# ETH3D/badslam

Measured on AMD Instinct MI355X. Metric: BA iterations/sec (and ms/iter) at N keyframes x M surfels, 640x480, higher is better.
Workload: dtype f32

## Files before the change

badslam_amd/csrc/kernels_surfel.hip:

```cpp
#include <stdlib.h>
#include <cstdio>

#include "ba_device.h"
#include "ba_launch.h"
#include "wave_cull.h"

namespace bahip {

#ifndef BAHIP_WAVES_ATTR
#define BAHIP_WAVES_ATTR __attribute__((amdgpu_waves_per_eu(4)))
#endif
constexpr int kSurfelBlock = 64;
constexpr int kMaxSumClasses = 8;

enum SumsMode { kSumsFused = 0, kSumsProduce = 1, kSumsConsume = 2 };
__device__ __forceinline__ bool position_valid(Vec3 p) { return p.x == p.x; }
static inline unsigned grid_for(uint32_t n) { return xcd_padded_tiles((n + kSurfelBlock - 1) / kSurfelBlock); }
#if defined(BAHIP_TILE_TIMELINE) && !defined(BAHIP_FAST_MATH)
__device__ unsigned long long g_geometry_timeline[65536][2];
void geometry_timeline_dump(const char* path) {
  static unsigned long long host[65536][2];
  if (hipMemcpyFromSymbol(host, HIP_SYMBOL(g_geometry_timeline), sizeof(host)) != hipSuccess) return;
  if (FILE* f = fopen(path, "wb")) { fwrite(host, sizeof(host), 1, f); fclose(f); }
}
#define BAHIP_RECORD_GEOMETRY_TIMELINE 1
#endif
}

BAHIP_FLAVOURED_BEGIN

template <int kWaves, int kCount, int kMode = kSumsFused, typename Visit>
__device__ __forceinline__ void tile_sums(float (&tot)[kCount], float* lds, Visit visit, int classes, const ClassPartials& cp = ClassPartials{},
                                          uint32_t i = 0, bool in_range = false) {
  static_assert(kWaves == 1 || kWaves == 2 || kWaves == 4, "1, 2 or 4 wavefronts per tile");
  static_assert(kMode == kSumsFused || kWaves == 1, "the class partials are exchanged by the one-wavefront shape only");
  if (kMode == kSumsProduce) {
#pragma nounroll
    for (int c = 0; c < classes; ++c) {
      if (!((cp.owned >> c) & 1u)) continue;
      float acc[kCount];
#pragma unroll
      for (int q = 0; q < kCount; ++q) acc[q] = 0.f;
      visit(acc, c);
      if (in_range) {
#pragma unroll
        for (int q = 0; q < kCount; ++q) cp.data[(size_t)(c * kCount + q) * cp.stride + i] = acc[q];
      }
    }
#pragma unroll
    for (int q = 0; q < kCount; ++q) tot[q] = 0.f;
  } else if (kMode == kSumsConsume) {
#pragma unroll
    for (int q = 0; q < kCount; ++q) {
      float t = cp.data[(size_t)(0 * kCount + q) * cp.stride + i] + cp.data[(size_t)(1 * kCount + q) * cp.stride + i];
      for (int c = 2; c < classes; ++c) t += cp.data[(size_t)(c * kCount + q) * cp.stride + i];
      tot[q] = t;
    }
  } else if (kWaves == 1) {
#pragma unroll
    for (int q = 0; q < kCount; ++q) tot[q] = 0.f;
#pragma nounroll
    for (int c = 0; c < classes; ++c) {
      float acc[kCount];
#pragma unroll
      for (int q = 0; q < kCount; ++q) acc[q] = 0.f;
      visit(acc, c);
#pragma unroll
      for (int q = 0; q < kCount; ++q) tot[q] += acc[q];
    }
  } else {
    const int part = threadIdx.x >> 6, lane = threadIdx.x & 63;
#pragma nounroll
    for (int c = part; c < classes; c += kWaves) {
      float acc[kCount];
#pragma unroll
      for (int q = 0; q < kCount; ++q) acc[q] = 0.f;
      visit(acc, c);
#pragma unroll
      for (int q = 0; q < kCount; ++q) lds[(c * kCount + q) * 64 + lane] = acc[q];
    }
    __syncthreads();
#pragma unroll
    for (int q = 0; q < kCount; ++q) {
      float t = lds[(0 * kCount + q) * 64 + lane] + lds[(1 * kCount + q) * 64 + lane];
      for (int c = 2; c < classes; ++c) t += lds[(c * kCount + q) * 64 + lane];
      tot[q] = t;
    }
    __syncthreads();
  }
}

__global__ void __launch_bounds__(kSurfelBlock) BAHIP_WAVES_ATTR
activation_kernel(Intrinsics in, const KfEntry* __restrict__ kfs, int num_kfs, SurfelsView s, uint32_t surfels_size) {
  const uint32_t i = xcd_chunked_tile(blockIdx.x) * kSurfelBlock + threadIdx.x;
  const bool in_range = i < surfels_size;
  const uint32_t ii = in_range ? i : 0;
  const Vec3 gp = surfel_position(s, ii);
  const Vec3 gn = surfel_normal(s, ii);
  const WaveBounds wb = wave_bounds(gp, in_range && position_valid(gp));
  bool active = false;
  for_each_candidate_until(
      num_kfs,
      [&](int k) { return kfs[k].activation == BAHIP_KF_ACTIVE && sphere_may_project(in, kfs[k].pose.F, wb); },
      [&](int k) {
        if (in_range && !active) {
          Assoc r;
          if (project_associate<false>(in, kfs[k].pose.F, kfs[k].geom, gp, gn, &r, nullptr)) active = true;
        }
        return __all(active || !in_range) != 0;
      });
  if (in_range) s.active[i] = (s.active[i] & (uint8_t)~kSurfelActiveFlag) | (active ? kSurfelActiveFlag : 0);
}

constexpr int kMaskChunks = 4;
template <int kWaves, bool kActivate, int kMode = kSumsFused>
__device__ __forceinline__ void normals_pass(const Intrinsics& in, const KfEntry* __restrict__ kfs, int num_kfs,
                                             const WaveBounds& wb, SurfelsView& s, uint32_t i, bool* live_inout, bool decide,
                                             Vec3 gp, Vec3* gn_inout, float* lds, const ClassPartials& cp = ClassPartials{},
                                             bool in_range = false, unsigned long long* masks = nullptr) {
  const bool writer = kWaves == 1 || (threadIdx.x >> 6) == 0;
  const Vec3 gn = *gn_inout;
  bool live = *live_inout;
  constexpr int kCount = kActivate ? 5 : 4;
  float sum[kCount];
  tile_sums<kWaves, kCount, kMode>(sum, lds, [&](float (&acc)[kCount], int cls) {
    struct Started { Projected p; PixelWords pix; };
    for_each_candidate_pipelined<Started>(
        num_kfs,
        [&](int k) {
          float f[12];
          int32_t activation;
          load_candidate(kfs[k].pose.F, &kfs[k].activation, f, &activation);
          return activation != BAHIP_KF_INACTIVE && sphere_may_project(in, f, wb);
        },
        [&](int k) {
          Started st;
          st.p = project_surfel(in, kfs[k].pose.F, gp);
          st.pix = load_pixel_words(in, kfs[k].geom, st.p);
          return st;
        },
        [&](int k, const Started& st) {
          const Projected& p = st.p;
          const PixelWords& pix = st.pix;
          Assoc r;
          const bool associated = live && associate_from_words<false>(in, kfs[k].pose.F, gn, p, pix, &r, nullptr);
          gathers_arrived(pix);
          if (associated) {
            const Vec3 g = mul33(kfs[k].pose.GR, unpack_normal8(r.normal_bits));
            acc[0] += g.x; acc[1] += g.y; acc[2] += g.z; acc[3] += 1.f;
            if (kActivate) acc[kCount - 1] += (kfs[k].activation == BAHIP_KF_ACTIVE) ? 1.f : 0.f;
          }
        },
        in.sum_classes, cls, masks ? masks + cls * kMaskChunks : nullptr, masks ? kMaskChunks : 0, false);
  }, in.sum_classes, cp, i, in_range);
  if (kMode == kSumsProduce) return;
  if (kActivate && decide) {
    const bool active = live && sum[kCount - 1] >= 1.f;
    if (writer) s.active[i] = (s.active[i] & (uint8_t)~kSurfelActiveFlag) | (active ? kSurfelActiveFlag : 0);
    live = active;
    *live_inout = active;
  }
  if (!live) return;
  const float sx = sum[0], sy = sum[1], sz = sum[2], count = sum[3];
  if (count >= 1) {
    const uint32_t packed = pack_normal10((1.f / count) * mk3(sx, sy, sz));
    if (writer) reinterpret_cast<uint32_t*>(s.row(kSurfelNormal))[i] = packed;
    *gn_inout = unpack_normal10(packed);
  }
}

template <int kWaves>
__global__ void __launch_bounds__(64 * kWaves) BAHIP_WAVES_ATTR
normals_kernel(Intrinsics in, const KfEntry* __restrict__ kfs, int num_kfs, SurfelsView s) {
  __shared__ float lds[kWaves == 1 ? 1 : kMaxSumClasses * 4 * 64];
  const int lane = threadIdx.x & 63;
  const uint32_t i = xcd_chunked_tile(blockIdx.x) * kSurfelBlock + lane;
  const bool in_range = i < s.size;
  const uint32_t ii = in_range ? i : 0;
  bool live = in_range && (s.active[ii] & kSurfelActiveFlag);
  const Vec3 gp = surfel_position(s, ii);
  Vec3 gn = surfel_normal(s, ii);
  const WaveBounds wb = wave_bounds(gp, live && position_valid(gp));
  normals_pass<kWaves, false>(in, kfs, num_kfs, wb, s, ii, &live, false, gp, &gn, lds);
}

template <bool kUseDepth, bool kUseDesc, int kWaves, bool kActivate, int kPhase>
__device__ __forceinline__ void geometry_step(const Intrinsics& in, const KfEntry* __restrict__ kfs, int num_kfs, SurfelsView& s,
                                              uint32_t activate_count, float* lds, const ClassPartials& cpn, const ClassPartials& cpp,
                                              uint32_t tile , unsigned long long* replay_masks) {
  constexpr int kNormalsMode = kPhase == 1 ? kSumsProduce : kPhase == 2 ? kSumsConsume : kSumsFused;
  constexpr int kPositionMode = kPhase == 2 ? kSumsProduce : kPhase == 3 ? kSumsConsume : kSumsFused;
  const int lane = threadIdx.x & 63;
  const bool writer = kWaves == 1 || (threadIdx.x >> 6) == 0;
  const uint32_t i = tile * kSurfelBlock + lane;
  const bool in_range = i < s.size;
  const uint32_t ii = in_range ? i : 0;
  const bool decide = kActivate && kPhase != 3 && in_range && i < activate_count;
  bool live = in_range && (decide || (s.active[ii] & kSurfelActiveFlag));
  const Vec3 gp = surfel_position(s, ii);
  Vec3 gn = surfel_normal(s, ii);
  const WaveBounds wb = wave_bounds(gp, live && position_valid(gp));
  if (wb.r < 0.f) {
    if (decide && writer && kPhase != 1) s.active[ii] = s.active[ii] & (uint8_t)~kSurfelActiveFlag;
    return;
  }
  constexpr bool kReplayMasks = kWaves == 1 && kPhase == 0;
  unsigned long long* masks = kReplayMasks ? replay_masks : nullptr;
  if (kPhase != 3) normals_pass<kWaves, kActivate, kNormalsMode>(in, kfs, num_kfs, wb, s, ii, &live, decide, gp, &gn, lds, cpn, in_range, masks);
  if (kPhase == 1) return;

  auto cand = [&](int k) {
    float f[12];
    int32_t activation;
    load_candidate(kfs[k].pose.F, &kfs[k].activation, f, &activation);
    return activation != BAHIP_KF_INACTIVE && sphere_may_project(in, f, wb);
  };

  if (!kUseDesc) {
    float hb[2];
    tile_sums<kWaves, 2, kPositionMode>(hb, lds, [&](float (&acc)[2], int cls) {
      for_each_candidate_cached(num_kfs, cand, [&](int k) {
        const Projected p = project_surfel(in, kfs[k].pose.F, gp);
        const PixelWords pix = load_pixel_words(in, kfs[k].geom, p);
        Assoc r;
        const bool associated = live && associate_from_words<false>(in, kfs[k].pose.F, gn, p, pix, &r, nullptr);
        gathers_arrived(pix);
        if (!associated) return;
        const float inv_std = assoc_inv_std(in, r);
        const float jac = -inv_std;
        const Vec3 u = assoc_unproject(r);
        const float raw = inv_std * dot3(r.nl, u - r.local);
        const float w = depth_residual_weight(raw);
        const float wj = w * jac;
        acc[0] = mad(wj, jac, acc[0]);
        acc[1] = mad(wj, raw, acc[1]);
      }, in.sum_classes, cls, masks ? masks + cls * kMaskChunks : nullptr, masks ? kMaskChunks : 0, masks != nullptr);
    }, in.sum_classes, cpp, ii, in_range);
    if (kPhase == 2 || !live || !writer) return;
    const float H = hb[0], b = hb[1];
    if (H > 1e-6f) {
      const float t = -1.f * b / H;
      const Vec3 np = gp + t * gn;
      s.row(kSurfelX)[i] = np.x; s.row(kSurfelY)[i] = np.y; s.row(kSurfelZ)[i] = np.z;
    }
    return;
  }

  const float radius_sq = s.row(kSurfelRadiusSquared)[ii];
  const float d1 = s.row(kSurfelDescriptor1)[ii];
  const float d2 = s.row(kSurfelDescriptor2)[ii];
  const TangentPoints tp = surfel_tangent_points(gp, gn, radius_sq);
  float tot[8];
  tile_sums<kWaves, 8, kPositionMode>(tot, lds, [&](float (&acc)[8], int cls) {
    float &a0 = acc[0], &a1 = acc[1], &a2 = acc[2], &a3 = acc[3], &a5 = acc[4], &a6 = acc[5], &a7 = acc[6], &a8 = acc[7];
    struct StartedPair { Projected p; PixelWords pix; };
    auto start_pair = [&](int k) {
      StartedPair st;
      st.p = project_surfel(in, kfs[k].pose.F, gp);
      st.pix = load_pixel_words(in, kfs[k].geom, st.p);
      return st;
    };
    auto finish_pair = [&](int k, const StartedPair& st) {
      const float* F = kfs[k].pose.F;
      const Projected& p = st.p;
      const PixelWords& pix = st.pix;
      const DescWords dw = load_descriptor_words(in, kfs[k].lumafp, F, tp, p);
      Assoc r;
      const bool associated = live && associate_from_words<false>(in, F, gn, p, pix, &r, nullptr);
#ifdef BAHIP_PIN_POSITION
      gathers_arrived(pix, dw);
#endif
      if (!associated) return;
      if (kUseDepth) {
        const float inv_std = assoc_inv_std(in, r);
        const float jac = -inv_std;
        const Vec3 u = assoc_unproject(r);
        const float raw = inv_std * dot3(r.nl, u - r.local);
        const float w = depth_residual_weight(raw);
        a0 = mad(w * jac, jac, a0);
        a6 = mad(w * raw, jac, a6);
      }
      if (dw.color_ok) {
        DescEval e;
        eval_descriptor_from_words(in, kfs[k].lumafp, dw, d1, d2, &e);
        const float jp1 = jac_descriptor_surfel(r.nl, r.local, r.inv_z, e.gx1, e.gy1, in.cfx, in.cfy);
        const float jp2 = jac_descriptor_surfel(r.nl, r.local, r.inv_z, e.gx2, e.gy2, in.cfx, in.cfy);
        const float jd = -1.f;
        const float w1 = descriptor_residual_weight(e.r1);
        const float wr1 = w1 * e.r1;
        const float w2 = descriptor_residual_weight(e.r2);
        const float wr2 = w2 * e.r2;
        a0 = mad(w2 * jp2, jp2, mad(w1 * jp1, jp1, a0));
        a1 += w1 * jp1 * jd;
        a3 += w1 * jd * jd;
        a6 = mad(wr2, jp2, mad(wr1, jp1, a6));
        a7 += wr1 * jd;
        a2 += w2 * jp2 * jd;
        a5 += w2 * jd * jd;
        a8 += wr2 * jd;
      }
    };
    if (kWaves == 1)
      for_each_candidate_pipelined<StartedPair>(num_kfs, cand, start_pair, finish_pair, in.sum_classes, cls, masks ? masks + cls * kMaskChunks : nullptr,
                                                masks ? kMaskChunks : 0, masks != nullptr);
    else
      for_each_candidate_cached(num_kfs, cand, [&](int k) { finish_pair(k, start_pair(k)); }, in.sum_classes, cls,
                                masks ? masks + cls * kMaskChunks : nullptr, masks ? kMaskChunks : 0, masks != nullptr);
  }, in.sum_classes, cpp, ii, in_range);
  if (kPhase == 2 || !live || !writer) return;
  const float a0 = tot[0], a1 = tot[1], a2 = tot[2], a3 = tot[3], a5 = tot[4], a6 = tot[5], a7 = tot[6], a8 = tot[7];

  float H00 = a0 + 1e-6f, H01 = a1, H02 = a2, H11 = a3 + 1e-6f, H12 = 0.f, H22 = a5 + 1e-6f;
  H00 = sqrtf(H00);
  H01 = H01 / H00;
  H11 = sqrtf(H11 - H01 * H01);
  H02 = H02 / H00;
  H12 = (H12 - H02 * H01) / H11;
  H22 = sqrtf(H22 - H02 * H02 - H12 * H12);
  const float y0 = a6 / H00;
  const float y1 = (a7 - H01 * y0) / H11;
  const float y2 = (a8 - H02 * y0 - H12 * y1) / H22;
  const float x2 = y2 / H22;
  const float x1 = (y1 - H12 * x2) / H11;
  const float x0 = (y0 - H02 * x2 - H01 * x1) / H00;
  if (x0 != 0) {
    const Vec3 np = gp - x0 * gn;
    s.row(kSurfelX)[i] = np.x; s.row(kSurfelY)[i] = np.y; s.row(kSurfelZ)[i] = np.z;
  }
  if (x1 != 0) s.row(kSurfelDescriptor1)[i] = fmaxf(-180.f, fminf(180.f, d1 - x1));
  if (x2 != 0) s.row(kSurfelDescriptor2)[i] = fmaxf(-180.f, fminf(180.f, d2 - x2));
}


template <bool kUseDepth, bool kUseDesc, int kWaves, bool kActivate>
__global__ void __launch_bounds__(64 * kWaves) BAHIP_WAVES_ATTR
geometry_kernel(Intrinsics in, const KfEntry* __restrict__ kfs, int num_kfs, SurfelsView s, uint32_t activate_count,
                const uint32_t* __restrict__ sched, const int* __restrict__ stop ) {
  __shared__ float lds[kWaves == 1 ? 1 : kMaxSumClasses * 8 * 64];
  __shared__ unsigned long long candidate_masks[kWaves == 1 ? kMaxSumClasses * kMaskChunks : 1];
  if (stop && load_global(stop) != 0) return;
#ifdef BAHIP_RECORD_GEOMETRY_TIMELINE
  const unsigned long long t0 = wall_clock64();
#endif
  uint32_t tile;
  if (!scheduled_tile(blockIdx.x, gridDim.x - (sched ? kHeavySlots : 0u), sched, &tile)) return;
  geometry_step<kUseDepth, kUseDesc, kWaves, kActivate, 0>(in, kfs, num_kfs, s, activate_count, lds, ClassPartials{}, ClassPartials{}, tile, candidate_masks);
#ifdef BAHIP_RECORD_GEOMETRY_TIMELINE
  if (threadIdx.x == 0 && blockIdx.x < 65536) { g_geometry_timeline[blockIdx.x][0] = t0; g_geometry_timeline[blockIdx.x][1] = wall_clock64(); }
#endif
}

#ifndef BAHIP_HYBRID_WAVES
#define BAHIP_HYBRID_WAVES 4
#endif
template <bool kUseDepth, bool kUseDesc, bool kActivate>
__global__ void __launch_bounds__(256) __attribute__((amdgpu_waves_per_eu(BAHIP_HYBRID_WAVES)))
geometry_hybrid_kernel(Intrinsics in, const KfEntry* __restrict__ kfs, int num_kfs, SurfelsView s, uint32_t activate_count,
                       const uint32_t* __restrict__ sched , uint32_t padded_tiles, const int* __restrict__ stop) {
  __shared__ float lds[kMaxSumClasses * 8 * 64];
  __shared__ unsigned long long candidate_masks[4][kMaxSumClasses * kMaskChunks];
  if (stop && load_global(stop) != 0) return;
  if (blockIdx.x < kHeavySlots) {
    if (blockIdx.x >= sched[0]) return;
    geometry_step<kUseDepth, kUseDesc, 4, kActivate, 0>(in, kfs, num_kfs, s, activate_count, lds, ClassPartials{}, ClassPartials{}, sched[8 + blockIdx.x], nullptr);
  } else {
    const uint32_t wave = threadIdx.x >> 6, position = (blockIdx.x - kHeavySlots) * 4u + wave;
    if (position >= padded_tiles) return;
    const uint32_t tile = (uint32_t)__builtin_amdgcn_readfirstlane((int)sched[kSchedPerm + position]);
    if (sched[kSchedPerm + padded_tiles + tile] != 0) return;
    geometry_step<kUseDepth, kUseDesc, 1, kActivate, 0>(in, kfs, num_kfs, s, activate_count, nullptr, ClassPartials{}, ClassPartials{}, tile, candidate_masks[wave]);
  }
}

template <bool kUseDepth, bool kUseDesc, bool kActivate, int kPhase>
__global__ void __launch_bounds__(64) BAHIP_WAVES_ATTR
geometry_phase_kernel(Intrinsics in, const KfEntry* __restrict__ kfs, int num_kfs, SurfelsView s, uint32_t activate_count,
                      ClassPartials cpn, ClassPartials cpp) {
  geometry_step<kUseDepth, kUseDesc, 1, kActivate, kPhase>(in, kfs, num_kfs, s, activate_count, nullptr, cpn, cpp, xcd_run_tile(blockIdx.x, gridDim.x), nullptr);
}

template <int kPhase>
__global__ void __launch_bounds__(kSurfelBlock) BAHIP_WAVES_ATTR
normals_phase_kernel(Intrinsics in, const KfEntry* __restrict__ kfs, int num_kfs, SurfelsView s, ClassPartials cp) {
  const uint32_t i = xcd_chunked_tile(blockIdx.x) * kSurfelBlock + threadIdx.x;
  const bool in_range = i < s.size;
  const uint32_t ii = in_range ? i : 0;
  bool live = in_range && (s.active[ii] & kSurfelActiveFlag);
  const Vec3 gp = surfel_position(s, ii);
  Vec3 gn = surfel_normal(s, ii);
  const WaveBounds wb = wave_bounds(gp, live && position_valid(gp));
  static_assert(kNormalsSums == 4, "normals_pass without activation: x, y, z, count");
  normals_pass<1, false, kPhase == 1 ? kSumsProduce : kSumsConsume>(in, kfs, num_kfs, wb, s, ii, &live, false, gp, &gn, nullptr, cp, in_range);
}

__global__ void __launch_bounds__(kSurfelBlock) BAHIP_WAVES_ATTR
activation_hits_kernel(Intrinsics in, const KfEntry* __restrict__ kfs, int num_kfs, SurfelsView s, uint32_t surfels_size,
                       uint32_t owner_mask, uint32_t owner_rank, uint32_t* __restrict__ hits) {
  const uint32_t i = xcd_chunked_tile(blockIdx.x) * kSurfelBlock + threadIdx.x;
  const bool in_range = i < surfels_size;
  const uint32_t ii = in_range ? i : 0;
  const Vec3 gp = surfel_position(s, ii);
  const Vec3 gn = surfel_normal(s, ii);
  const WaveBounds wb = wave_bounds(gp, in_range && position_valid(gp));
  bool active = false;
  for_each_candidate_until(
      num_kfs,
      [&](int k) {
        return ((uint32_t)k & owner_mask) == owner_rank && kfs[k].activation == BAHIP_KF_ACTIVE && sphere_may_project(in, kfs[k].pose.F, wb);
      },
      [&](int k) {
        if (in_range && !active) {
          Assoc r;
          if (project_associate<false>(in, kfs[k].pose.F, kfs[k].geom, gp, gn, &r, nullptr)) active = true;
        }
        return __all(active || !in_range) != 0;
      });
  if (in_range) hits[i] = active ? 1u : 0u;
}
void launch_activation(hipStream_t stream, const Intrinsics& in, const KfEntry* kfs, int num_kfs, const SurfelsView& s,
                       uint32_t surfels_size) {
  if (surfels_size == 0) return;
  hipLaunchKernelGGL(activation_kernel, dim3(grid_for(surfels_size)), dim3(kSurfelBlock), 0, stream, in, kfs, num_kfs, s,
                     surfels_size);
}

static int g_forced_tile_waves = bahip_env_int("BAHIP_TILE_WAVES", 0);
static long long g_geometry_hybrid_launches = 0;
long long geometry_hybrid_launches() { return g_geometry_hybrid_launches; }
void set_tile_waves(int waves) { g_forced_tile_waves = waves; }
static int tile_waves(uint32_t surfels) {
  const int forced = g_forced_tile_waves;
  if (forced == 1 || forced == 4) return forced;
  return grid_for(surfels) >= 8192 ? 1 : 4;
}

void launch_normals(hipStream_t stream, const Intrinsics& in, const KfEntry* kfs, int num_kfs, const SurfelsView& s) {
  if (s.size == 0) return;
  const dim3 grid(grid_for(s.size));
  switch (tile_waves(s.size)) {
    case 1: hipLaunchKernelGGL(normals_kernel<1>, grid, dim3(64), 0, stream, in, kfs, num_kfs, s); break;
    default: hipLaunchKernelGGL(normals_kernel<4>, grid, dim3(256), 0, stream, in, kfs, num_kfs, s); break;
  }
}

template <int kWaves, bool kActivate>
static void launch_geometry_shape(hipStream_t stream, bool use_depth, bool use_desc, const Intrinsics& in, const KfEntry* kfs,
                                  int num_kfs, const SurfelsView& s, uint32_t activate_count, const uint32_t* sched, const int* stop) {
  const dim3 grid(sched_positions(grid_for(s.size), sched)), block(64 * kWaves);
  if (!use_desc) hipLaunchKernelGGL((geometry_kernel<true, false, kWaves, kActivate>), grid, block, 0, stream, in, kfs, num_kfs, s, activate_count, sched, stop);
  else if (use_depth) hipLaunchKernelGGL((geometry_kernel<true, true, kWaves, kActivate>), grid, block, 0, stream, in, kfs, num_kfs, s, activate_count, sched, stop);
  else hipLaunchKernelGGL((geometry_kernel<false, true, kWaves, kActivate>), grid, block, 0, stream, in, kfs, num_kfs, s, activate_count, sched, stop);
}

template <bool kActivate>
static void launch_geometry_hybrid(hipStream_t stream, bool use_depth, bool use_desc, const Intrinsics& in, const KfEntry* kfs,
                                   int num_kfs, const SurfelsView& s, uint32_t activate_count, const uint32_t* sched, const int* stop) {
  const uint32_t padded = grid_for(s.size);
  const dim3 grid(kHeavySlots + (padded + 3u) / 4u), block(256);
  if (!use_desc) hipLaunchKernelGGL((geometry_hybrid_kernel<true, false, kActivate>), grid, block, 0, stream, in, kfs, num_kfs, s, activate_count, sched, padded, stop);
  else if (use_depth) hipLaunchKernelGGL((geometry_hybrid_kernel<true, true, kActivate>), grid, block, 0, stream, in, kfs, num_kfs, s, activate_count, sched, padded, stop);
  else hipLaunchKernelGGL((geometry_hybrid_kernel<false, true, kActivate>), grid, block, 0, stream, in, kfs, num_kfs, s, activate_count, sched, padded, stop);
}

void launch_geometry(hipStream_t stream, bool use_depth, bool use_desc, const Intrinsics& in, const KfEntry* kfs,
                     int num_kfs, const SurfelsView& s, long long activate_count, const uint32_t* sched, const int* stop) {
  if (s.size == 0) return;
  const uint32_t n = activate_count < 0 ? 0u : (uint32_t)activate_count;
  const bool hybrid = sched != nullptr && (g_forced_tile_waves == 5 || (g_forced_tile_waves == 0 && grid_for(s.size) < 8192));
  if (hybrid) {
    ++g_geometry_hybrid_launches;
    if (activate_count < 0) launch_geometry_hybrid<false>(stream, use_depth, use_desc, in, kfs, num_kfs, s, n, sched, stop);
    else launch_geometry_hybrid<true>(stream, use_depth, use_desc, in, kfs, num_kfs, s, n, sched, stop);
  } else if (tile_waves(s.size) == 1) {
    if (activate_count < 0) launch_geometry_shape<1, false>(stream, use_depth, use_desc, in, kfs, num_kfs, s, n, sched, stop);
    else launch_geometry_shape<1, true>(stream, use_depth, use_desc, in, kfs, num_kfs, s, n, sched, stop);
  } else {
    if (activate_count < 0) launch_geometry_shape<4, false>(stream, use_depth, use_desc, in, kfs, num_kfs, s, n, sched, stop);
    else launch_geometry_shape<4, true>(stream, use_depth, use_desc, in, kfs, num_kfs, s, n, sched, stop);
  }
}

template <bool kUseDepth, bool kUseDesc, bool kActivate>
static void launch_geometry_phase_of(hipStream_t stream, int phase, const Intrinsics& in, const KfEntry* kfs, int num_kfs, const SurfelsView& s,
                                     uint32_t activate_count, const ClassPartials& cpn, const ClassPartials& cpp) {
  const dim3 grid(grid_for(s.size)), block(64);
  if (phase == 1) hipLaunchKernelGGL((geometry_phase_kernel<kUseDepth, kUseDesc, kActivate, 1>), grid, block, 0, stream, in, kfs, num_kfs, s, activate_count, cpn, cpp);
  else if (phase == 2) hipLaunchKernelGGL((geometry_phase_kernel<kUseDepth, kUseDesc, kActivate, 2>), grid, block, 0, stream, in, kfs, num_kfs, s, activate_count, cpn, cpp);
  else hipLaunchKernelGGL((geometry_phase_kernel<kUseDepth, kUseDesc, kActivate, 3>), grid, block, 0, stream, in, kfs, num_kfs, s, activate_count, cpn, cpp);
}

void launch_geometry_phase(hipStream_t stream, int phase, bool use_depth, bool use_desc, const Intrinsics& in, const KfEntry* kfs, int num_kfs,
                           const SurfelsView& s, long long activate_count, const ClassPartials& cpn, const ClassPartials& cpp) {
  if (s.size == 0) return;
  const uint32_t n = activate_count < 0 ? 0u : (uint32_t)activate_count;
  const bool act = activate_count >= 0;
  if (!use_desc) {
    if (act) launch_geometry_phase_of<true, false, true>(stream, phase, in, kfs, num_kfs, s, n, cpn, cpp);
    else launch_geometry_phase_of<true, false, false>(stream, phase, in, kfs, num_kfs, s, n, cpn, cpp);
  } else if (use_depth) {
    if (act) launch_geometry_phase_of<true, true, true>(stream, phase, in, kfs, num_kfs, s, n, cpn, cpp);
    else launch_geometry_phase_of<true, true, false>(stream, phase, in, kfs, num_kfs, s, n, cpn, cpp);
  } else {
    if (act) launch_geometry_phase_of<false, true, true>(stream, phase, in, kfs, num_kfs, s, n, cpn, cpp);
    else launch_geometry_phase_of<false, true, false>(stream, phase, in, kfs, num_kfs, s, n, cpn, cpp);
  }
}

void launch_normals_phase(hipStream_t stream, int phase, const Intrinsics& in, const KfEntry* kfs, int num_kfs, const SurfelsView& s, const ClassPartials& cp) {
  if (s.size == 0) return;
  const dim3 grid(grid_for(s.size)), block(kSurfelBlock);
  if (phase == 1) hipLaunchKernelGGL(normals_phase_kernel<1>, grid, block, 0, stream, in, kfs, num_kfs, s, cp);
  else hipLaunchKernelGGL(normals_phase_kernel<2>, grid, block, 0, stream, in, kfs, num_kfs, s, cp);
}

void launch_activation_hits(hipStream_t stream, const Intrinsics& in, const KfEntry* kfs, int num_kfs, const SurfelsView& s, uint32_t surfels_size,
                            int kf_rank, int kf_world, uint32_t* hits) {
  if (surfels_size == 0) return;
  hipLaunchKernelGGL(activation_hits_kernel, dim3(grid_for(surfels_size)), dim3(kSurfelBlock), 0, stream, in, kfs, num_kfs, s, surfels_size,
                     (uint32_t)(kf_world - 1), (uint32_t)kf_rank, hits);
}
BAHIP_FLAVOURED_END

#ifndef BAHIP_FAST_MATH
namespace bahip {
__device__ __forceinline__ void sample_rgba(const uint8_t* color, uint32_t pitch, int w, int h, float x, float y, float (&out)[4]) {
  float xb = x - 0.5f, yb = y - 0.5f;
  if (!(xb >= -1.f)) xb = -1.f;
  if (xb > (float)w) xb = (float)w;
  if (!(yb >= -1.f)) yb = -1.f;
  if (yb > (float)h) yb = (float)h;
  const float fx = floorf(xb), fy = floorf(yb);
  const float a = xb - fx, b = yb - fy;
  const int x0 = min(max((int)fx, 0), w - 1), x1 = min(max((int)fx + 1, 0), w - 1);
  const int y0 = min(max((int)fy, 0), h - 1), y1 = min(max((int)fy + 1, 0), h - 1);
  const uchar4* image = reinterpret_cast<const uchar4*>(color);
  const uchar4 tl = pitched_load(image, pitch, y0, x0), tr = pitched_load(image, pitch, y0, x1);
  const uchar4 bl = pitched_load(image, pitch, y1, x0), br = pitched_load(image, pitch, y1, x1);
  const uint8_t ctl[4] = {tl.x, tl.y, tl.z, tl.w}, ctr[4] = {tr.x, tr.y, tr.z, tr.w};
  const uint8_t cbl[4] = {bl.x, bl.y, bl.z, bl.w}, cbr[4] = {br.x, br.y, br.z, br.w};
#pragma unroll
  for (int c = 0; c < 4; ++c) {
    const float vtl = (float)ctl[c] * (1.0f / 255.0f), vtr = (float)ctr[c] * (1.0f / 255.0f);
    const float vbl = (float)cbl[c] * (1.0f / 255.0f), vbr = (float)cbr[c] * (1.0f / 255.0f);
    const float top = mad(a, vtr - vtl, vtl);
    const float bot = mad(a, vbr - vbl, vbl);
    out[c] = mad(b, bot - top, top);
  }
}

__global__ void __launch_bounds__(kSurfelBlock) BAHIP_WAVES_ATTR
assign_colors_kernel(Intrinsics in, const KfEntry* __restrict__ kfs, int num_kfs, SurfelsView s) {
  const uint32_t i = xcd_chunked_tile(blockIdx.x) * kSurfelBlock + threadIdx.x;
  const bool in_range = i < s.size;
  const uint32_t ii = in_range ? i : 0;
  const Vec3 gp = surfel_position(s, ii);
  const Vec3 gn = surfel_normal(s, ii);
  const WaveBounds wb = wave_bounds(gp, in_range && position_valid(gp));
  float count = 0.f, sum[4] = {0.f, 0.f, 0.f, 0.f};
  for_each_candidate(
      num_kfs, [&](int k) { return sphere_may_project_item(in, kfs[k].pose.F, wb); },
      [&](int k) {
        if (!in_range) return;
        Assoc r;
        if (!project_associate<false>(in, kfs[k].pose.F, kfs[k].geom, gp, gn, &r, nullptr)) return;
        float cx, cy;
        if (!depth_to_color_pixel(in, r.pxx, r.pxy, &cx, &cy)) return;
        float c[4];
        sample_rgba(kfs[k].color, kfs[k].color_pitch, in.cwidth, in.cheight, cx, cy, c);
        count += 1.f;
#pragma unroll
        for (int q = 0; q < 4; ++q) sum[q] += c[q];
      });
  if (in_range && count > 0.f) {
    uchar4 out;
    out.x = (uint8_t)(255.f * sum[0] / count + 0.5f);
    out.y = (uint8_t)(255.f * sum[1] / count + 0.5f);
    out.z = (uint8_t)(255.f * sum[2] / count + 0.5f);
    out.w = (uint8_t)(255.f * sum[3] / count + 0.5f);
    reinterpret_cast<uchar4*>(s.row(kSurfelColor))[i] = out;
  }
}

__global__ void activation_from_hits_kernel(SurfelsView s, uint32_t surfels_size, const uint32_t* __restrict__ hits) {
  const uint32_t i = blockIdx.x * blockDim.x + threadIdx.x;
  if (i < surfels_size) s.active[i] = (s.active[i] & (uint8_t)~kSurfelActiveFlag) | (hits[i] ? kSurfelActiveFlag : 0);
}

void launch_assign_colors(hipStream_t stream, const Intrinsics& in, const KfEntry* kfs, int num_kfs, const SurfelsView& s) {
  if (s.size == 0) return;
  hipLaunchKernelGGL(assign_colors_kernel, dim3(grid_for(s.size)), dim3(kSurfelBlock), 0, stream, in, kfs, num_kfs, s);
}

int geometry_normals_sums(bool activate) { return activate ? 5 : 4; }
int geometry_position_sums(bool use_desc) { return use_desc ? 8 : 2; }
void launch_activation_from_hits(hipStream_t stream, const SurfelsView& s, uint32_t surfels_size, const uint32_t* hits) {
  if (surfels_size == 0) return;
  hipLaunchKernelGGL(activation_from_hits_kernel, dim3((surfels_size + 255) / 256), dim3(256), 0, stream, s, surfels_size, hits);
}


void launch_activation(hipStream_t stream, const Intrinsics& in, const KfEntry* kfs, int num_kfs, const SurfelsView& s, uint32_t surfels_size) {
  BAHIP_PICK(in, launch_activation(stream, in, kfs, num_kfs, s, surfels_size));
}
void launch_normals(hipStream_t stream, const Intrinsics& in, const KfEntry* kfs, int num_kfs, const SurfelsView& s) {
  BAHIP_PICK(in, launch_normals(stream, in, kfs, num_kfs, s));
}
void launch_geometry(hipStream_t stream, bool use_depth, bool use_desc, const Intrinsics& in, const KfEntry* kfs, int num_kfs, const SurfelsView& s,
                     long long activate_count, const uint32_t* sched, const int* stop) {
  BAHIP_PICK(in, launch_geometry(stream, use_depth, use_desc, in, kfs, num_kfs, s, activate_count, sched, stop));
}
void launch_geometry_phase(hipStream_t stream, int phase, bool use_depth, bool use_desc, const Intrinsics& in, const KfEntry* kfs, int num_kfs,
                           const SurfelsView& s, long long activate_count, const ClassPartials& cpn, const ClassPartials& cpp) {
  BAHIP_PICK(in, launch_geometry_phase(stream, phase, use_depth, use_desc, in, kfs, num_kfs, s, activate_count, cpn, cpp));
}
void launch_normals_phase(hipStream_t stream, int phase, const Intrinsics& in, const KfEntry* kfs, int num_kfs, const SurfelsView& s, const ClassPartials& cp) {
  BAHIP_PICK(in, launch_normals_phase(stream, phase, in, kfs, num_kfs, s, cp));
}
void launch_activation_hits(hipStream_t stream, const Intrinsics& in, const KfEntry* kfs, int num_kfs, const SurfelsView& s, uint32_t surfels_size,
                            int kf_rank, int kf_world, uint32_t* hits) {
  BAHIP_PICK(in, launch_activation_hits(stream, in, kfs, num_kfs, s, surfels_size, kf_rank, kf_world, hits));
}
void set_tile_waves(int waves) { exact::set_tile_waves(waves); fast::set_tile_waves(waves); }
long long geometry_hybrid_launches() { return exact::geometry_hybrid_launches() + fast::geometry_hybrid_launches(); }
}

namespace bahip {
__global__ void __launch_bounds__(kSurfelBlock) BAHIP_WAVES_ATTR
count_pairs_kernel(Intrinsics in, const KfEntry* __restrict__ kfs, int num_kfs, SurfelsView s, unsigned long long* counts) {
  const uint32_t i = xcd_chunked_tile(blockIdx.x) * kSurfelBlock + threadIdx.x;
  const bool in_range = i < s.size;
  const uint32_t ii = in_range ? i : 0;
  const Vec3 gp = surfel_position(s, ii);
  const Vec3 gn = surfel_normal(s, ii);
  const WaveBounds wb = wave_bounds(gp, in_range && position_valid(gp));
  unsigned long long cand = 0, wave_hits = 0, lane_hits = 0, in_image = 0;
  for_each_candidate(
      num_kfs, [&](int k) { return sphere_may_project_item(in, kfs[k].pose.F, wb); },
      [&](int k) {
        Assoc r;
        const bool hit = in_range && project_associate<false>(in, kfs[k].pose.F, kfs[k].geom, gp, gn, &r, nullptr);
        const Vec3 l = transform34(kfs[k].pose.F, gp);
        const float px = mad(in.fx, l.x * (1.f / l.z), in.cx), py = mad(in.fy, l.y * (1.f / l.z), in.cy);
        const bool inside = in_range && l.z > 0 && px >= 0 && py >= 0 && px < in.width && py < in.height;
        const unsigned long long m = __ballot(hit);
        cand += 1; wave_hits += (m != 0); lane_hits += __popcll(m); in_image += __popcll(__ballot(inside));
      });
  if ((threadIdx.x & 63) == 0) {
    atomicAdd(&counts[0], cand); atomicAdd(&counts[1], wave_hits); atomicAdd(&counts[2], lane_hits); atomicAdd(&counts[3], in_image);
  }
}
void launch_count_pairs(hipStream_t stream, const Intrinsics& in, const KfEntry* kfs, int num_kfs, const SurfelsView& s,
                        unsigned long long* counts) {
  if (s.size) hipLaunchKernelGGL(count_pairs_kernel, dim3(grid_for(s.size)), dim3(kSurfelBlock), 0, stream, in, kfs, num_kfs, s, counts);
}
}
#endif
```

Baseline: 745.3.

## Park geometry-step loop-invariant state in LDS to raise single-wave occupancy

In the one-wavefront geometry kernel with descriptors, the wave bounds, tangent points, normal, descriptors and the running class totals are moved into per-lane LDS slots. They are reloaded inside the candidate loops, with asm barriers that stop the compiler from keeping them in VGPRs. The waves-per-EU target for that kernel is raised from 4 to 5, aiming to fit under the tighter register budget without scratch spills. The cost is extra LDS traffic and reloads on every candidate keyframe, plus more LDS per workgroup.

```diff
diff --git a/badslam_amd/csrc/kernels_surfel.hip b/badslam_amd/csrc/kernels_surfel.hip
--- a/badslam_amd/csrc/kernels_surfel.hip
+++ b/badslam_amd/csrc/kernels_surfel.hip
@@ -10,10 +10,32 @@
 #ifndef BAHIP_WAVES_ATTR
 #define BAHIP_WAVES_ATTR __attribute__((amdgpu_waves_per_eu(4)))
 #endif
+#ifndef BAHIP_GEOMETRY_WAVES
+#define BAHIP_GEOMETRY_WAVES 5
+#endif
+#if BAHIP_GEOMETRY_WAVES > 5
+#warning "BAHIP_GEOMETRY_WAVES > 5: the parked state (ParkSlot) does not bring the joint solve under 80 VGPRs; expect 10-13 dwords of scratch per lane"
+#endif
 constexpr int kSurfelBlock = 64;
 constexpr int kMaxSumClasses = 8;
 
 enum SumsMode { kSumsFused = 0, kSumsProduce = 1, kSumsConsume = 2 };
+
+enum ParkSlot {
+  kParkTotals = 0,
+  kParkTangents = 8,
+  kParkDesc = 14,
+  kParkBounds = 16,
+  kParkNormal = 20,
+  kParkSlots = 23
+};
+constexpr int kMaskChunks = 4;
+static_assert((kParkSlots * 64 * 4 + kMaxSumClasses * kMaskChunks * 8) * 4 * BAHIP_GEOMETRY_WAVES <= 160 * 1024, "parked state: LDS per workgroup");
+typedef __attribute__((address_space(3))) float ParkedFloat;
+__device__ __forceinline__ ParkedFloat* park_lane(float* block) { return (ParkedFloat*)block + (threadIdx.x & 63); }
+__device__ __forceinline__ void park_reopen(ParkedFloat*& lane) { asm volatile("" : "+v"(lane)); }
+__device__ __forceinline__ void park_put(ParkedFloat* lane, int slot, float v) { lane[slot * 64] = v; }
+__device__ __forceinline__ float park_get(ParkedFloat* lane, int slot) { return lane[slot * 64]; }
 __device__ __forceinline__ bool position_valid(Vec3 p) { return p.x == p.x; }
 static inline unsigned grid_for(uint32_t n) { return xcd_padded_tiles((n + kSurfelBlock - 1) / kSurfelBlock); }
 #if defined(BAHIP_TILE_TIMELINE) && !defined(BAHIP_FAST_MATH)
@@ -88,6 +110,28 @@
     }
     __syncthreads();
   }
+}
+
+template <int kCount, typename Visit>
+__device__ __forceinline__ void tile_sums_parked(float (&tot)[kCount], ParkedFloat*& park, int slot, Visit visit, int classes) {
+#pragma unroll
+  for (int q = 0; q < kCount; ++q) park_put(park, slot + q, 0.f);
+#pragma nounroll
+  for (int c = 0; c < classes; ++c) {
+    float acc[kCount];
+#pragma unroll
+    for (int q = 0; q < kCount; ++q) acc[q] = 0.f;
+    visit(acc, c);
+    park_reopen(park);
+    float t[kCount];
+#pragma unroll
+    for (int q = 0; q < kCount; ++q) t[q] = park_get(park, slot + q);
+#pragma unroll
+    for (int q = 0; q < kCount; ++q) park_put(park, slot + q, t[q] + acc[q]);
+  }
+  park_reopen(park);
+#pragma unroll
+  for (int q = 0; q < kCount; ++q) tot[q] = park_get(park, slot + q);
 }
 
 __global__ void __launch_bounds__(kSurfelBlock) BAHIP_WAVES_ATTR
@@ -112,7 +156,6 @@
   if (in_range) s.active[i] = (s.active[i] & (uint8_t)~kSurfelActiveFlag) | (active ? kSurfelActiveFlag : 0);
 }
 
-constexpr int kMaskChunks = 4;
 template <int kWaves, bool kActivate, int kMode = kSumsFused>
 __device__ __forceinline__ void normals_pass(const Intrinsics& in, const KfEntry* __restrict__ kfs, int num_kfs,
                                              const WaveBounds& wb, SurfelsView& s, uint32_t i, bool* live_inout, bool decide,
@@ -184,10 +227,12 @@
   normals_pass<kWaves, false>(in, kfs, num_kfs, wb, s, ii, &live, false, gp, &gn, lds);
 }
 
-template <bool kUseDepth, bool kUseDesc, int kWaves, bool kActivate, int kPhase>
+template <bool kUseDepth, bool kUseDesc, int kWaves, bool kActivate, int kPhase, bool kPark = false>
 __device__ __forceinline__ void geometry_step(const Intrinsics& in, const KfEntry* __restrict__ kfs, int num_kfs, SurfelsView& s,
                                               uint32_t activate_count, float* lds, const ClassPartials& cpn, const ClassPartials& cpp,
-                                              uint32_t tile , unsigned long long* replay_masks) {
+                                              uint32_t tile , unsigned long long* replay_masks,
+                                              float* park_block = nullptr) {
+  static_assert(!kPark || (kWaves == 1 && kPhase == 0), "state is parked by the one-wavefront kernel of the whole step only");
   constexpr int kNormalsMode = kPhase == 1 ? kSumsProduce : kPhase == 2 ? kSumsConsume : kSumsFused;
   constexpr int kPositionMode = kPhase == 2 ? kSumsProduce : kPhase == 3 ? kSumsConsume : kSumsFused;
   const int lane = threadIdx.x & 63;
@@ -209,11 +254,28 @@
   if (kPhase != 3) normals_pass<kWaves, kActivate, kNormalsMode>(in, kfs, num_kfs, wb, s, ii, &live, decide, gp, &gn, lds, cpn, in_range, masks);
   if (kPhase == 1) return;
 
+  constexpr bool kParked = kPark && kUseDesc;
+  ParkedFloat* park = nullptr;
+  if constexpr (kParked) {
+    park = park_lane(park_block);
+    park_put(park, kParkBounds + 0, wb.cx); park_put(park, kParkBounds + 1, wb.cy);
+    park_put(park, kParkBounds + 2, wb.cz); park_put(park, kParkBounds + 3, wb.r);
+  }
   auto cand = [&](int k) {
     float f[12];
     int32_t activation;
     load_candidate(kfs[k].pose.F, &kfs[k].activation, f, &activation);
-    return activation != BAHIP_KF_INACTIVE && sphere_may_project(in, f, wb);
+    if constexpr (kParked) {
+      park_reopen(park);
+      WaveBounds b;
+      b.cx = park_get(park, kParkBounds + 0); b.cy = park_get(park, kParkBounds + 1);
+      b.cz = park_get(park, kParkBounds + 2); b.r = park_get(park, kParkBounds + 3);
+      Intrinsics opaque = in;
+      asm volatile("" : "+s"(opaque.fx), "+s"(opaque.fy), "+s"(opaque.cx), "+s"(opaque.cy), "+s"(opaque.width), "+s"(opaque.height));
+      return activation != BAHIP_KF_INACTIVE && sphere_may_project(opaque, f, b);
+    } else {
+      return activation != BAHIP_KF_INACTIVE && sphere_may_project(in, f, wb);
+    }
   };
 
   if (!kUseDesc) {
@@ -250,8 +312,39 @@
   const float d1 = s.row(kSurfelDescriptor1)[ii];
   const float d2 = s.row(kSurfelDescriptor2)[ii];
   const TangentPoints tp = surfel_tangent_points(gp, gn, radius_sq);
+  if constexpr (kParked) {
+    park_put(park, kParkTangents + 0, tp.q1.x); park_put(park, kParkTangents + 1, tp.q1.y); park_put(park, kParkTangents + 2, tp.q1.z);
+    park_put(park, kParkTangents + 3, tp.q2.x); park_put(park, kParkTangents + 4, tp.q2.y); park_put(park, kParkTangents + 5, tp.q2.z);
+    park_put(park, kParkDesc + 0, d1); park_put(park, kParkDesc + 1, d2);
+    park_put(park, kParkNormal + 0, gn.x); park_put(park, kParkNormal + 1, gn.y); park_put(park, kParkNormal + 2, gn.z);
+  }
+  auto tangents = [&](TangentPoints& back) -> const TangentPoints& {
+    if constexpr (kParked) {
+      back.q1 = mk3(park_get(park, kParkTangents + 0), park_get(park, kParkTangents + 1), park_get(park, kParkTangents + 2));
+      back.q2 = mk3(park_get(park, kParkTangents + 3), park_get(park, kParkTangents + 4), park_get(park, kParkTangents + 5));
+      return back;
+    } else {
+      return tp;
+    }
+  };
+  auto normal = [&](Vec3& back) -> const Vec3& {
+    if constexpr (kParked) {
+      back = mk3(park_get(park, kParkNormal + 0), park_get(park, kParkNormal + 1), park_get(park, kParkNormal + 2));
+      return back;
+    } else {
+      return gn;
+    }
+  };
+  auto descriptors = [&](float (&back)[2]) -> const float* {
+    if constexpr (kParked) {
+      back[0] = park_get(park, kParkDesc + 0); back[1] = park_get(park, kParkDesc + 1);
+      return back;
+    } else {
+      return nullptr;
+    }
+  };
   float tot[8];
-  tile_sums<kWaves, 8, kPositionMode>(tot, lds, [&](float (&acc)[8], int cls) {
+  auto position_visit = [&](float (&acc)[8], int cls) {
     float &a0 = acc[0], &a1 = acc[1], &a2 = acc[2], &a3 = acc[3], &a5 = acc[4], &a6 = acc[5], &a7 = acc[6], &a8 = acc[7];
     struct StartedPair { Projected p; PixelWords pix; };
     auto start_pair = [&](int k) {
@@ -264,9 +357,14 @@
       const float* F = kfs[k].pose.F;
       const Projected& p = st.p;
       const PixelWords& pix = st.pix;
-      const DescWords dw = load_descriptor_words(in, kfs[k].lumafp, F, tp, p);
+      if constexpr (kParked) park_reopen(park);
+      TangentPoints tp_back;
+      Vec3 gn_back;
+      const TangentPoints& tpk = tangents(tp_back);
+      const Vec3& gnk = normal(gn_back);
+      const DescWords dw = load_descriptor_words(in, kfs[k].lumafp, F, tpk, p);
       Assoc r;
-      const bool associated = live && associate_from_words<false>(in, F, gn, p, pix, &r, nullptr);
+      const bool associated = live && associate_from_words<false>(in, F, gnk, p, pix, &r, nullptr);
 #ifdef BAHIP_PIN_POSITION
       gathers_arrived(pix, dw);
 #endif
@@ -282,7 +380,10 @@
       }
       if (dw.color_ok) {
         DescEval e;
-        eval_descriptor_from_words(in, kfs[k].lumafp, dw, d1, d2, &e);
+        if constexpr (kParked) park_reopen(park);
+        float d_back[2];
+        const float* dk = descriptors(d_back);
+        eval_descriptor_from_words(in, kfs[k].lumafp, dw, dk ? dk[0] : d1, dk ? dk[1] : d2, &e);
         const float jp1 = jac_descriptor_surfel(r.nl, r.local, r.inv_z, e.gx1, e.gy1, in.cfx, in.cfy);
         const float jp2 = jac_descriptor_surfel(r.nl, r.local, r.inv_z, e.gx2, e.gy2, in.cfx, in.cfy);
         const float jd = -1.f;
@@ -306,7 +407,9 @@
     else
       for_each_candidate_cached(num_kfs, cand, [&](int k) { finish_pair(k, start_pair(k)); }, in.sum_classes, cls,
                                 masks ? masks + cls * kMaskChunks : nullptr, masks ? kMaskChunks : 0, masks != nullptr);
-  }, in.sum_classes, cpp, ii, in_range);
+  };
+  if constexpr (kParked) tile_sums_parked<8>(tot, park, kParkTotals, position_visit, in.sum_classes);
+  else tile_sums<kWaves, 8, kPositionMode>(tot, lds, position_visit, in.sum_classes, cpp, ii, in_range);
   if (kPhase == 2 || !live || !writer) return;
   const float a0 = tot[0], a1 = tot[1], a2 = tot[2], a3 = tot[3], a5 = tot[4], a6 = tot[5], a7 = tot[6], a8 = tot[7];
 
@@ -323,28 +426,39 @@
   const float x2 = y2 / H22;
   const float x1 = (y1 - H12 * x2) / H11;
   const float x0 = (y0 - H02 * x2 - H01 * x1) / H00;
+  uint32_t iu = i;
+  if constexpr (kParked) {
+    iu = tile * kSurfelBlock + __lane_id();
+    park_reopen(park);
+  }
+  Vec3 gn_back;
+  float d_back[2];
+  const Vec3& gnu = normal(gn_back);
+  const float* du = descriptors(d_back);
+  const float d1u = du ? du[0] : d1, d2u = du ? du[1] : d2;
   if (x0 != 0) {
-    const Vec3 np = gp - x0 * gn;
-    s.row(kSurfelX)[i] = np.x; s.row(kSurfelY)[i] = np.y; s.row(kSurfelZ)[i] = np.z;
-  }
-  if (x1 != 0) s.row(kSurfelDescriptor1)[i] = fmaxf(-180.f, fminf(180.f, d1 - x1));
-  if (x2 != 0) s.row(kSurfelDescriptor2)[i] = fmaxf(-180.f, fminf(180.f, d2 - x2));
+    const Vec3 np = gp - x0 * gnu;
+    s.row(kSurfelX)[iu] = np.x; s.row(kSurfelY)[iu] = np.y; s.row(kSurfelZ)[iu] = np.z;
+  }
+  if (x1 != 0) s.row(kSurfelDescriptor1)[iu] = fmaxf(-180.f, fminf(180.f, d1u - x1));
+  if (x2 != 0) s.row(kSurfelDescriptor2)[iu] = fmaxf(-180.f, fminf(180.f, d2u - x2));
 }
 
 
 template <bool kUseDepth, bool kUseDesc, int kWaves, bool kActivate>
-__global__ void __launch_bounds__(64 * kWaves) BAHIP_WAVES_ATTR
+__global__ void __launch_bounds__(64 * kWaves) __attribute__((amdgpu_waves_per_eu(kWaves == 1 ? BAHIP_GEOMETRY_WAVES : 4)))
 geometry_kernel(Intrinsics in, const KfEntry* __restrict__ kfs, int num_kfs, SurfelsView s, uint32_t activate_count,
                 const uint32_t* __restrict__ sched, const int* __restrict__ stop ) {
   __shared__ float lds[kWaves == 1 ? 1 : kMaxSumClasses * 8 * 64];
   __shared__ unsigned long long candidate_masks[kWaves == 1 ? kMaxSumClasses * kMaskChunks : 1];
+  __shared__ float parked[kWaves == 1 ? kParkSlots * 64 : 1];
   if (stop && load_global(stop) != 0) return;
 #ifdef BAHIP_RECORD_GEOMETRY_TIMELINE
   const unsigned long long t0 = wall_clock64();
 #endif
   uint32_t tile;
   if (!scheduled_tile(blockIdx.x, gridDim.x - (sched ? kHeavySlots : 0u), sched, &tile)) return;
-  geometry_step<kUseDepth, kUseDesc, kWaves, kActivate, 0>(in, kfs, num_kfs, s, activate_count, lds, ClassPartials{}, ClassPartials{}, tile, candidate_masks);
+  geometry_step<kUseDepth, kUseDesc, kWaves, kActivate, 0, kWaves == 1>(in, kfs, num_kfs, s, activate_count, lds, ClassPartials{}, ClassPartials{}, tile, candidate_masks, parked);
 #ifdef BAHIP_RECORD_GEOMETRY_TIMELINE
   if (threadIdx.x == 0 && blockIdx.x < 65536) { g_geometry_timeline[blockIdx.x][0] = t0; g_geometry_timeline[blockIdx.x][1] = wall_clock64(); }
 #endif
```

Result: faster. 766.8 (median of 6 runs) (+2.9%).
